# fab-jul/imgcomp-cvpr

Hardware: AMD Instinct MI355X
Metric: Megapixels/s encode+pc-logits (and decode) per node (higher is better)
Workload: dtype f32

## Files before the change

### imgcomp_cvpr_amd/csrc/conv3x3_wino4.hip

```cpp
#include "wino_common.h"
#include "internal.h"

#define W4_QUADS 9
#define W4_PACKED_FLOATS (36 * WN_C * WN_C)
#define W4_ACC_A 32
#ifndef W4_RA
#define W4_RA 9
#endif
#ifndef W4_RB
#define W4_RB 3
#endif
#ifndef W4_TURN
#define W4_TURN 6
#endif
#ifndef W4_GAP
#define W4_GAP 10
#endif
#ifndef W4_PRE_N
#define W4_PRE_N 2
#endif
#ifndef W4_PRE
#define W4_PRE 31
#endif
#ifndef W4_WT_MAX
#define W4_WT_MAX 512
#endif
#ifndef W4_ABL
#define W4_ABL 0
#endif
#ifndef W4_SLICE1
#define W4_SLICE1 1
#endif
#ifndef W4_SOFT
#define W4_SOFT 0
#endif
#ifndef W4_WG8_FLAGS
#define W4_WG8_FLAGS 1
#endif
#define W4_WG8_SPINS (1 << 16)
#define W4_B1 29
#define W4_B2 8
#ifndef W4_SPREAD
#define W4_SPREAD 1
#endif

__device__ __forceinline__ int w4_tap5(int mode, int phase, int a) {
    if (mode == 2) return phase ? 2 * a : (a == 0 ? -1 : 2 * a - 1);
    return phase ? 4 - 2 * a : (a == 2 ? -1 : 3 - 2 * a);
}
__global__ __launch_bounds__(256) void wino4_pack_kernel(const float* __restrict__ w_tf, const float* const* __restrict__ w_tab, float* __restrict__ out,
                                                        int mode, int CI, int CO) {
    const int idx = blockIdx.x * 256 + threadIdx.x;
    if (idx >= CI * CO) return;
    if (w_tab) { w_tf = w_tab[blockIdx.y]; out += (size_t)blockIdx.y * 36 * CI * CO; }
    const int cin = idx / CO, cout = idx % CO;
    double g[3][3];
#pragma unroll
    for (int a = 0; a < 3; ++a)
#pragma unroll
        for (int b = 0; b < 3; ++b) {
            if (mode == 0) g[a][b] = (double)w_tf[((a * 3 + b) * WN_C + cin) * WN_C + cout];
            else if (mode == 1) g[a][b] = (double)w_tf[(((2 - a) * 3 + (2 - b)) * WN_C + cout) * WN_C + cin];
            else if (mode == 2) {
                const int ph = cin >> 6, c = cin & 63, ky = w4_tap5(2, ph >> 1, a), kx = w4_tap5(2, ph & 1, b);
                g[a][b] = (ky < 0 || kx < 0) ? 0.0 : (double)w_tf[((ky * 5 + kx) * 64 + c) * 128 + cout];
            } else {
                const int ph = cout & 3, c = cout >> 2, ky = w4_tap5(3, ph >> 1, a), kx = w4_tap5(3, ph & 1, b);
                g[a][b] = (ky < 0 || kx < 0) ? 0.0 : (double)w_tf[((ky * 5 + kx) * 64 + c) * 128 + cin];
            }
        }
    const double G[6][3] = {{0.25, 0.0, 0.0}, {-1.0 / 6, -1.0 / 6, -1.0 / 6}, {-1.0 / 6, 1.0 / 6, -1.0 / 6},
                            {1.0 / 24, 1.0 / 12, 1.0 / 6}, {1.0 / 24, -1.0 / 12, 1.0 / 6}, {0.0, 0.0, 1.0}};
    double t[6][3];
#pragma unroll
    for (int x = 0; x < 6; ++x)
#pragma unroll
        for (int b = 0; b < 3; ++b) t[x][b] = G[x][0] * g[0][b] + G[x][1] * g[1][b] + G[x][2] * g[2][b];
    float* o = out + ((size_t)((cout >> 4) * (CI >> 2) + (cin >> 2)) * W4_QUADS * 64 + ((cin & 3) * 16 + (cout & 15))) * 4;
#pragma unroll
    for (int x = 0; x < 6; ++x)
#pragma unroll
        for (int v = 0; v < 6; ++v) {
            const int p = 6 * x + v;
            o[(p >> 2) * 256 + (p & 3)] = (float)(t[x][0] * G[v][0] + t[x][1] * G[v][1] + t[x][2] * G[v][2]);
        }
}

extern "C" size_t ic_wino4_3x3_c128_packed_floats(void) { return W4_PACKED_FLOATS; }

extern "C" int ic_pack_wino4_3x3_c128_f32(const float* w_tf, float* w_packed, int backward, ic_stream_t stream) {
    IC_CHECK_ARG(w_tf && w_packed);
    hipLaunchKernelGGL(wino4_pack_kernel, dim3(WN_C * WN_C / 256), dim3(256), 0, (hipStream_t)stream, w_tf, nullptr, w_packed, backward ? 1 : 0, WN_C, WN_C);
    IC_LAUNCH_CHECK();
    return IC_OK;
}

extern "C" int ic_pack_wino4_3x3_c128_batch_f32(const float* const* w_tf_table_dev, float* w_packed, int layers, int backward, ic_stream_t stream) {
    IC_CHECK_ARG(w_tf_table_dev && w_packed && layers > 0);
    hipLaunchKernelGGL(wino4_pack_kernel, dim3(WN_C * WN_C / 256, layers), dim3(256), 0, (hipStream_t)stream, nullptr, w_tf_table_dev, w_packed,
                       backward ? 1 : 0, WN_C, WN_C);
    IC_LAUNCH_CHECK();
    return IC_OK;
}

extern "C" size_t ic_wino4_conv5s2_packed_floats(void) { return (size_t)36 * 256 * 128; }

extern "C" int ic_pack_wino4_conv5s2_f32(const float* w_tf, float* w_packed, int transposed, ic_stream_t stream) {
    IC_CHECK_ARG(w_tf && w_packed);
    hipLaunchKernelGGL(wino4_pack_kernel, dim3(256 * 128 / 256), dim3(256), 0, (hipStream_t)stream, w_tf, nullptr, w_packed, transposed ? 3 : 2,
                       transposed ? 128 : 256, transposed ? 256 : 128);
    IC_LAUNCH_CHECK();
    return IC_OK;
}

__device__ __forceinline__ void w4_bt(const float d0, const float d1, const float d2, const float d3, const float d4, const float d5,
                                      float& t0, float& t1, float& t2, float& t3, float& t4, float& t5) {
    const float p = fmaf(-4.f, d2, d4), q = fmaf(-4.f, d1, d3);
    const float r = d4 - d2, s = 2.f * (d3 - d1);
    const float a0 = fmaf(4.f, d0, fmaf(-5.f, d2, d4));
    const float a5 = fmaf(4.f, d1, fmaf(-5.f, d3, d5));
    t0 = a0;
    t1 = p + q;
    t2 = p - q;
    t3 = r + s;
    t4 = r - s;
    t5 = a5;
}
__device__ __forceinline__ void w4_at(float m0, float m1, float m2, float m3, float m4, float m5,
                                      float& y0, float& y1, float& y2, float& y3) {
    const float s1 = m1 + m2, d1 = m1 - m2, s2 = m3 + m4, d2 = m3 - m4;
    y0 = (m0 + s1) + s2;
    y1 = fmaf(2.f, d2, d1);
    y2 = fmaf(4.f, s2, s1);
    y3 = fmaf(8.f, d2, d1) + m5;
}

template <bool WT, int RES, int CIN, int COUT, bool SHUF, bool SEG2, bool WG8, bool STATS = false>
__global__ __launch_bounds__(WG8 ? 512 : 256) __attribute__((amdgpu_waves_per_eu(2, 2)))
void wino4_3x3_kernel(const WnArgs a) {
    constexpr int WAVES = WG8 ? 8 : 4;
    constexpr int KS = CIN / 4, IT = KS / 4, PARTS = COUT / (16 * WAVES);
    __shared__ f32x4 ring[2 * 4 * W4_QUADS * 64];
    __shared__ float pf_sink[64];
    __shared__ unsigned w8_flag[4];
#ifdef W4_STAMPS
    const unsigned long long t_entry = __builtin_amdgcn_s_memtime();
#endif
#ifdef W4_LAUNCH_STAMPS
    const unsigned long long ls_c0 = __builtin_amdgcn_s_memtime(), ls_r0 = __builtin_amdgcn_s_memrealtime();
#endif
    const int wave = __builtin_amdgcn_readfirstlane(threadIdx.x >> 6);
    const int lane = threadIdx.x & 63, n16 = lane & 15, kq = lane >> 4;
    const int b = a.xcd_runs ? ic_xcd_run(blockIdx.x, gridDim.x) : (int)blockIdx.x;
    const int part = b % PARTS;
    const int seg = b / PARTS + a.g0;
    const int sx = seg % a.gcols, t_ = seg / a.gcols;
    const int ty = t_ % a.grows, n = t_ / a.grows;
    const int cot = part * WAVES + wave;
    const int pw = wave & 3;
    const int grp = WG8 ? wave >> 2 : 0;
    const int hrow = SEG2 ? (n16 >> 3) : 0;
    const int tx = SEG2 ? 8 * sx + (n16 & 7) : 16 * sx + n16;
    const int H = a.H, W = a.W, HW = H * W;

    const __amdgpu_buffer_rsrc_t xr = __builtin_amdgcn_make_buffer_rsrc((void*)(a.x + (size_t)n * CIN * HW), 0, CIN * HW * 4, 0x00020000);
    const __amdgpu_buffer_rsrc_t fr = __builtin_amdgcn_make_buffer_rsrc((void*)a.wp, 0, 36 * CIN * COUT * 4, 0x00020000);
    const bool col_ok = 4 * tx < W;
    const bool first_lane = SEG2 ? (n16 & 7) == 0 : n16 == 0, last_lane = SEG2 ? (n16 & 7) == 7 : n16 == 15;
    const bool mid_l = SEG2 && n16 == 8, mid_r = SEG2 && n16 == 7;
    const int ecol = first_lane ? 4 * tx - 1 : (last_lane ? 4 * tx + 4 : -1);
    const bool e_ok = col_ok && ecol >= 0 && ecol < W;
    const int tyr = SEG2 ? 2 * ty : ty;
    const int r_first = 4 * tyr - 1;
    const int obase = (kq * HW + (r_first + 4 * hrow) * W + 4 * tx) * 4;
    const int ebase = (kq * HW + (r_first + 4 * hrow) * W + ecol) * 4;
    const unsigned fo = (unsigned)lane * 16u;

    f32x4 acc[36];
#pragma unroll
    for (int p = 0; p < 36; ++p) acc[p] = f32x4{0.f, 0.f, 0.f, 0.f};
#pragma unroll
    for (int p = 0; p < 36; ++p) {
        if (p < W4_ACC_A) asm volatile("" : "+a"(acc[p]));
        else asm volatile("" : "+v"(acc[p]));
    }
    __builtin_amdgcn_sched_barrier(0);

    typedef __attribute__((address_space(3))) f32x4 lds_f32x4;
    unsigned rb1 = (unsigned)(size_t)&ring[4 * W4_QUADS * 64 + lane];
    if (WG8) asm volatile("" : "+v"(rb1));
    auto ring_rd = [&](int half, int idx) __attribute__((always_inline)) -> f32x4 {
        if (WG8 && half) return *(reinterpret_cast<lds_f32x4*>((size_t)rb1) + idx * 64);
        return ring[(half * 4 * W4_QUADS + idx) * 64 + lane];
    };

    f32x4 pr[6];
    float pe[6];
    auto load_patch = [&](int ks) __attribute__((always_inline)) {
        const int so = ks * 4 * HW * 4;
        int ob = obase, eb = ebase;
        asm volatile("" : "+v"(ob), "+v"(eb));
#pragma unroll
        for (int i = 0; i < 6; ++i) {
            const bool row_lo = r_first + i >= 0 && r_first + i < H;
            const bool row_hi = r_first + 4 + i < H;
            const bool row_ok = SEG2 ? (hrow ? row_hi : row_lo) : row_lo;
            const unsigned o1 = (row_ok && col_ok) ? (unsigned)(ob + i * W * 4) : WN_OOB;
            const unsigned o2 = (row_ok && e_ok) ? (unsigned)(eb + i * W * 4) : WN_OOB;
            pr[i] = __builtin_bit_cast(f32x4, __builtin_amdgcn_raw_buffer_load_b128(xr, o1, so, 0));
            pe[i] = __builtin_bit_cast(float, __builtin_amdgcn_raw_buffer_load_b32(xr, o2, so, 0));
        }
    };
    auto transform_put = [&](int half) __attribute__((always_inline)) {
        float u[6][6];
#pragma unroll
        for (int i = 0; i < 6; ++i) {
            u[i][0] = dpp_from_left(pe[i], pr[i][3]);
            u[i][5] = dpp_from_right(pe[i], pr[i][0]);
            if (SEG2) { u[i][0] = mid_l ? pe[i] : u[i][0]; u[i][5] = mid_r ? pe[i] : u[i][5]; }
            u[i][1] = pr[i][0]; u[i][2] = pr[i][1]; u[i][3] = pr[i][2]; u[i][4] = pr[i][3];
        }
        __builtin_amdgcn_sched_barrier(0);
#pragma unroll
        for (int j = 0; j < 6; ++j) {
            w4_bt(u[0][j], u[1][j], u[2][j], u[3][j], u[4][j], u[5][j], u[0][j], u[1][j], u[2][j], u[3][j], u[4][j], u[5][j]);
            __builtin_amdgcn_sched_barrier(0);
        }
        f32x4* dst = &ring[((half * 4 + pw) * W4_QUADS) * 64 + lane];
#pragma unroll
        for (int x = 0; x < 6; x += 2) {
            float v0[6], v1[6];
            w4_bt(u[x][0], u[x][1], u[x][2], u[x][3], u[x][4], u[x][5], v0[0], v0[1], v0[2], v0[3], v0[4], v0[5]);
            w4_bt(u[x + 1][0], u[x + 1][1], u[x + 1][2], u[x + 1][3], u[x + 1][4], u[x + 1][5], v1[0], v1[1], v1[2], v1[3], v1[4], v1[5]);
            const int q0 = 3 * (x / 2);
            dst[(q0 + 0) * 64] = f32x4{v0[0], v0[1], v0[2], v0[3]};
            dst[(q0 + 1) * 64] = f32x4{v0[4], v0[5], v1[0], v1[1]};
            dst[(q0 + 2) * 64] = f32x4{v1[2], v1[3], v1[4], v1[5]};
            __builtin_amdgcn_sched_barrier(0);
        }
    };
    float su[6][6], sp = 0.f, sq = 0.f, sr = 0.f, se = 0.f, sa = 0.f, sh4 = 0.f, sh5 = 0.f;
    auto bt_first = [&](float d0, float d1, float d2, float d3, float d4) __attribute__((always_inline)) {
        sp = fmaf(-4.f, d2, d4); sq = fmaf(-4.f, d1, d3); sr = d4 - d2; se = d3 - d1;
        sa = fmaf(4.f, d0, fmaf(-5.f, d2, d4));
    };
    auto bt_second = [&](float d1, float d3, float d5, float& t0, float& t1, float& t2, float& t3, float& t4, float& t5) __attribute__((always_inline)) {
        const float a5 = fmaf(4.f, d1, fmaf(-5.f, d3, d5));
        t0 = sa; t1 = sp + sq; t2 = sp - sq; t3 = fmaf(2.f, se, sr); t4 = fmaf(-2.f, se, sr); t5 = a5;
    };
    auto slice = [&](int k, int part, int half) __attribute__((always_inline)) {
        if (k == 0) {
#pragma unroll
            for (int i = 0; i < 6; ++i) {
                if (part == 0) {
                    su[i][0] = dpp_from_left(pe[i], pr[i][3]);
                    if (SEG2) su[i][0] = mid_l ? pe[i] : su[i][0];
                } else {
                    su[i][5] = dpp_from_right(pe[i], pr[i][0]);
                    if (SEG2) su[i][5] = mid_r ? pe[i] : su[i][5];
                    su[i][1] = pr[i][0]; su[i][2] = pr[i][1]; su[i][3] = pr[i][2]; su[i][4] = pr[i][3];
                }
            }
        } else if (k <= 6) {
            const int c = k == 1 ? 0 : (k == 2 ? 5 : k - 2);
            if (part == 0) bt_first(su[0][c], su[1][c], su[2][c], su[3][c], su[4][c]);
            else bt_second(su[1][c], su[3][c], su[5][c], su[0][c], su[1][c], su[2][c], su[3][c], su[4][c], su[5][c]);
        } else {
            const int x = k - 7;
            if (part == 0) bt_first(su[x][0], su[x][1], su[x][2], su[x][3], su[x][4]);
            else {
                float v[6];
                bt_second(su[x][1], su[x][3], su[x][5], v[0], v[1], v[2], v[3], v[4], v[5]);
                f32x4* dst = &ring[((half * 4 + pw) * W4_QUADS + 3 * (x / 2)) * 64 + lane];
                if ((x & 1) == 0) { dst[0] = f32x4{v[0], v[1], v[2], v[3]}; sh4 = v[4]; sh5 = v[5]; }
                else { dst[64] = f32x4{sh4, sh5, v[0], v[1]}; dst[128] = f32x4{v[2], v[3], v[4], v[5]}; }
            }
        }
    };
    auto kill_patch = [&]() __attribute__((always_inline)) {
#pragma unroll
        for (int i = 0; i < 6; ++i) { asm volatile("" : "=v"(pr[i])); asm volatile("" : "=v"(pe[i])); }
    };
    auto kill_slices = [&]() __attribute__((always_inline)) {
#pragma unroll
        for (int i = 0; i < 6; ++i)
#pragma unroll
            for (int jx = 0; jx < 6; ++jx) asm volatile("" : "=v"(su[i][jx]));
        asm volatile("" : "=v"(sp)); asm volatile("" : "=v"(sq)); asm volatile("" : "=v"(sr)); asm volatile("" : "=v"(se));
        asm volatile("" : "=v"(sa)); asm volatile("" : "=v"(sh4)); asm volatile("" : "=v"(sh5));
    };
    const unsigned w8_base = (unsigned)(size_t)w8_flag;
    auto flag_add = [&](int k) __attribute__((always_inline)) {
        asm volatile("s_mov_b64 exec, 1\n\tds_add_u32 %0, %1\n\ts_mov_b64 exec, -1" :: "v"(w8_base + 4u * k), "v"(1u) : "memory");
    };
    auto flag_wait = [&](int k, unsigned target) __attribute__((always_inline)) {
        unsigned v, sv, spins;
        asm volatile("s_mov_b32 %2, 0\n"
                     "1:\tds_read_b32 %0, %3\n\t"
                     "s_waitcnt lgkmcnt(0)\n\t"
                     "v_readfirstlane_b32 %1, %0\n\t"
                     "s_add_u32 %2, %2, 1\n\t"
                     "s_cmp_ge_u32 %1, %4\n\t"
                     "s_cbranch_scc1 2f\n\t"
                     "s_cmp_lt_u32 %2, %5\n\t"
                     "s_cbranch_scc1 1b\n"
                     "2:"
                     : "=&v"(v), "=&s"(sv), "=&s"(spins) : "v"(w8_base + 4u * k), "s"(target), "i"(W4_WG8_SPINS) : "memory", "scc");
    };
    f32x4 fa[W4_RA];
    auto load_filter = [&](int slot, int Q) __attribute__((always_inline)) {
        fa[slot] = __builtin_bit_cast(f32x4, __builtin_amdgcn_raw_buffer_load_b128(fr, fo, (cot * KS * W4_QUADS + Q) * 1024, 0));
    };

    const int img_bytes = COUT * HW * 4;
    f32x4 e1a[4], e1b[4];
    float scv[4], shv[4];
#pragma unroll
    for (int i = 0; i < 4; ++i) { e1a[i] = e1b[i] = f32x4{0.f, 0.f, 0.f, 0.f}; scv[i] = shv[i] = 0.f; }
    auto epilogue_lanes = [&](unsigned* lo, int& kq_e) __attribute__((always_inline)) {
        int lane_e = (int)__builtin_amdgcn_mbcnt_hi(~0u, __builtin_amdgcn_mbcnt_lo(~0u, 0u));
        asm volatile("" : "+v"(lane_e));
        kq_e = lane_e >> 4;
        const int tx_e = SEG2 ? 8 * sx + (lane_e & 7) : 16 * sx + (lane_e & 15);
        const bool col_ok_e = 4 * tx_e < W;
#pragma unroll
        for (int i = 0; i < 4; ++i) {
            const int oy = 4 * (SEG2 ? 2 * ty + ((lane_e >> 3) & 1) : ty) + i;
            lo[i] = (col_ok_e && oy < H) ? (unsigned)((4 * kq_e * HW + oy * W + 4 * tx_e) * 4) : WN_OOB;
        }
    };
    auto request_first = [&](int first, int count) __attribute__((always_inline)) {
        unsigned lo[4];
        int kq_e;
        epilogue_lanes(lo, kq_e);
        if (first == 0 && !STATS) {
#pragma unroll
            for (int r = 0; r < 4; ++r) {
                const int ch = SHUF ? 4 * cot + kq_e : 16 * cot + 4 * kq_e + r;
                scv[r] = a.scale[ch]; shv[r] = a.shift[ch];
            }
        }
        if (RES > 0) {
            const __amdgpu_buffer_rsrc_t r1r = __builtin_amdgcn_make_buffer_rsrc((void*)(a.res1 ? a.res1 + (size_t)n * COUT * HW : a.x), 0, a.res1 ? img_bytes : 0, 0x00020000);
#pragma unroll
            for (int i = 0; i < 4; ++i) {
                if (first == 0) e1a[i] = __builtin_bit_cast(f32x4, __builtin_amdgcn_raw_buffer_load_b128(r1r, lo[i], 16 * cot * HW * 4, 0));
                if (first + count > 1) e1b[i] = __builtin_bit_cast(f32x4, __builtin_amdgcn_raw_buffer_load_b128(r1r, lo[i], (16 * cot + 1) * HW * 4, 0));
            }
        }
    };

    if (!WG8 || grp == 0) load_patch(pw);
#pragma unroll
    for (int Q = 0; Q < W4_RA - 1; ++Q) load_filter(Q, Q);
    if (a.wp_next) {
        constexpr unsigned LINES = 36u * CIN * COUT * 4u / 128u;
        const unsigned n_x = (gridDim.x + 7u) >> 3, j_x = blockIdx.x >> 3;
        const unsigned per = (LINES + n_x - 1) / n_x, l0 = j_x * per;
        const __amdgpu_buffer_rsrc_t nr = __builtin_amdgcn_make_buffer_rsrc((void*)a.wp_next, 0, 36 * CIN * COUT * 4, 0x00020000);
        const unsigned sink = (unsigned)(size_t)pf_sink;
        for (unsigned l = threadIdx.x; l < per; l += 64 * WAVES) {
            const unsigned off = (l0 + l) < LINES ? (l0 + l) * 128u : WN_OOB;
            unsigned keep;
            asm volatile("s_mov_b32 %0, m0\n\ts_mov_b32 m0, %3\n\ts_nop 0\n\tbuffer_load_dword %1, %2, 0 offen lds\n\ts_mov_b32 m0, %0"
                         : "=&s"(keep) : "v"(off), "s"(nr), "s"(sink) : "memory");
        }
    }
    if (!WG8 || grp == 0) transform_put(0);
    if (WG8 && W4_WG8_FLAGS && threadIdx.x < 4) w8_flag[threadIdx.x] = 0u;
    asm volatile("s_waitcnt lgkmcnt(0)" ::: "memory");
    __builtin_amdgcn_s_barrier();

#ifdef W4_STAMPS
    const unsigned long long t_loop0 = __builtin_amdgcn_s_memtime();
#endif
    f32x4 bq[W4_RB];
#pragma unroll
    for (int q0 = 0; q0 < W4_RB - 1; ++q0) bq[q0] = ring_rd(0, q0);
    auto iteration = [&](const int j, const int u2, const bool last, const bool produce) __attribute__((always_inline)) {
        if (WG8 && W4_WG8_FLAGS && j > 0) flag_wait(u2, 4u * ((unsigned)(j + 1) >> 1));
        if (!W4_SOFT && j > 0) {
#pragma unroll
            for (int q0 = 0; q0 < W4_RB - 1; ++q0) bq[q0] = ring_rd(u2, q0);
        }
#pragma unroll
        for (int lq = 0; lq < 36; ++lq) {
            const int q = lq % W4_QUADS;
            const int Q = j * 36 + lq;
            const int sk = lq - (W4_TURN + W4_GAP);
#pragma unroll
            for (int i = 0; i < 4; ++i) {
                if (4 * q + i < W4_ACC_A) asm volatile("v_mfma_f32_16x16x4_f32 %0, %1, %2, %0" : "+a"(acc[4 * q + i]) : "v"(fa[lq % W4_RA][i]), "v"(bq[lq % W4_RB][i]));
                else asm volatile("v_mfma_f32_16x16x4_f32 %0, %1, %2, %0" : "+v"(acc[4 * q + i]) : "v"(fa[lq % W4_RA][i]), "v"(bq[lq % W4_RB][i]));
                if (WG8 && !last && sk == 0 && i == 0) kill_slices();
                if (W4_SPREAD && produce && !(W4_ABL & 4) && i < (W4_SLICE1 ? 1 : 2) && sk >= 0 && sk < 13) {
                    __builtin_amdgcn_sched_barrier(0);
                    if (WG8 && W4_WG8_FLAGS && sk == 7 && i == 0) flag_wait(2 + (u2 ^ 1), 8u * ((unsigned)(j + 1) >> 1));
                    slice(sk, i, u2 ^ 1);
                    if (W4_SLICE1) slice(sk, 1, u2 ^ 1);
                    if (WG8 && W4_WG8_FLAGS && sk == 12 && i == (W4_SLICE1 ? 0 : 1)) flag_add(u2 ^ 1);
                    __builtin_amdgcn_sched_barrier(0);
                }
            }
#if W4_ABL & 1
            if ((lq & 1) == 0)
#endif
            if (!last || lq + W4_RA - 1 < 36) load_filter((lq + W4_RA - 1) % W4_RA, Q + W4_RA - 1);
            {
                const int ah = lq + W4_RB - 1;
                if (ah < 36 && !((W4_ABL & 2) && (lq & 1)))
                    bq[ah % W4_RB] = ring_rd(u2, ah);
                else if (W4_SOFT && !last) bq[ah % W4_RB] = ring_rd(u2 ^ 1, ah - 36);
            }
            if (WG8 && !last && lq == W4_TURN) kill_patch();
            if (lq == W4_TURN && produce) load_patch(4 * (j + 1) + pw);
            if (!W4_SPREAD && lq == W4_TURN + W4_GAP && produce) transform_put(u2 ^ 1);
            if (last && lq == W4_PRE) request_first(0, W4_PRE_N);
            if (W4_SOFT && !last && lq == W4_B1) {
                asm volatile("s_waitcnt lgkmcnt(0)" ::: "memory");
                __builtin_amdgcn_s_barrier();
            }
            if (W4_SOFT && !last && lq == W4_B2 && j > 0) __builtin_amdgcn_s_barrier();
            if (WG8 && W4_WG8_FLAGS && !last && lq == 36 - W4_RB + 1) flag_add(2 + u2);
            __builtin_amdgcn_sched_barrier(0);
        }
        if (!W4_SOFT && !(WG8 && W4_WG8_FLAGS)) {
            asm volatile("s_waitcnt lgkmcnt(0)" ::: "memory");
            __builtin_amdgcn_s_barrier();
        }
    };
    for (int jj = 0; jj < IT - 2; jj += 2) {
        iteration(jj, 0, false, !WG8 || grp == 1);
        iteration(jj + 1, 1, false, !WG8 || grp == 0);
    }
    iteration(IT - 2, 0, false, !WG8 || grp == 1);
    iteration(IT - 1, 1, true, false);
#ifdef W4_STAMPS
    const unsigned long long t_loop1 = __builtin_amdgcn_s_memtime();
#endif

    asm volatile("s_nop 15\n\ts_nop 15" ::: "memory");
#pragma unroll
    for (int p = 0; p < 36; ++p) {
        if (p < W4_ACC_A) asm volatile("" : "+a"(acc[p]));
        else asm volatile("" : "+v"(acc[p]));
    }

    if (W4_PRE < 0) request_first(0, 2);
    else if (W4_PRE_N < 2) request_first(1, 1);
    unsigned lo[4];
    int kq_e;
    epilogue_lanes(lo, kq_e);
    const float relu_lo = a.relu ? 0.f : -__builtin_inff();
    auto out_tile = [&](int r, float (&y)[4][4]) __attribute__((always_inline)) {
        float w_[6][4];
#pragma unroll
        for (int x = 0; x < 6; ++x) {
#pragma unroll
            for (int v = 0; v < 6; ++v) {
                if (6 * x + v < W4_ACC_A) asm volatile("" : "+a"(acc[6 * x + v]));
                else asm volatile("" : "+v"(acc[6 * x + v]));
            }
            w4_at(acc[6 * x][r], acc[6 * x + 1][r], acc[6 * x + 2][r], acc[6 * x + 3][r], acc[6 * x + 4][r], acc[6 * x + 5][r],
                  w_[x][0], w_[x][1], w_[x][2], w_[x][3]);
            __builtin_amdgcn_sched_barrier(0);
        }
#pragma unroll
        for (int jx = 0; jx < 4; ++jx) {
            w4_at(w_[0][jx], w_[1][jx], w_[2][jx], w_[3][jx], w_[4][jx], w_[5][jx], y[0][jx], y[1][jx], y[2][jx], y[3][jx]);
            __builtin_amdgcn_sched_barrier(0);
        }
    };
    if (SHUF) {
        const __amdgpu_buffer_rsrc_t yr = __builtin_amdgcn_make_buffer_rsrc((void*)(a.y + (size_t)n * COUT * HW), 0, img_bytes, 0x00020000);
        int lane_s = (int)__builtin_amdgcn_mbcnt_hi(~0u, __builtin_amdgcn_mbcnt_lo(~0u, 0u));
        asm volatile("" : "+v"(lane_s));
        const int tx_s = SEG2 ? 8 * sx + (lane_s & 7) : 16 * sx + (lane_s & 15);
        const int ty_s = SEG2 ? 2 * ty + ((lane_s >> 3) & 1) : ty;
        const bool col_ok_s = 4 * tx_s < W;
        const int so = 4 * cot * 4 * HW * 4;
#pragma unroll
        for (int py = 0; py < 2; ++py) {
            f32x4 o0[4], o1[4];
            {
                float y[4][4];
                out_tile(2 * py, y);
#pragma unroll
                for (int i = 0; i < 4; ++i) {
#pragma unroll
                    for (int jx = 0; jx < 4; ++jx) o0[i][jx] = fmaxf(fmaf(y[i][jx], scv[0], shv[0]), relu_lo);
                    asm volatile("" : "+v"(o0[i]));
                }
            }
            __builtin_amdgcn_sched_barrier(0);
            {
                float y[4][4];
                out_tile(2 * py + 1, y);
#pragma unroll
                for (int i = 0; i < 4; ++i) {
#pragma unroll
                    for (int jx = 0; jx < 4; ++jx) o1[i][jx] = fmaxf(fmaf(y[i][jx], scv[0], shv[0]), relu_lo);
                }
            }
            __builtin_amdgcn_sched_barrier(0);
#pragma unroll
            for (int i = 0; i < 4; ++i) {
                const int oy = 4 * ty_s + i;
                const unsigned lo_s = (col_ok_s && oy < H) ? (unsigned)(((lane_s >> 4) * 4 * HW + (2 * oy + py) * 2 * W + 8 * tx_s) * 4) : WN_OOB;
                const f32x4 oa = f32x4{o0[i][0], o1[i][0], o0[i][1], o1[i][1]}, ob = f32x4{o0[i][2], o1[i][2], o0[i][3], o1[i][3]};
                __builtin_amdgcn_raw_buffer_store_b128(__builtin_bit_cast(u32x4, oa), yr, lo_s, so, WT ? 16 : 0);
                __builtin_amdgcn_raw_buffer_store_b128(__builtin_bit_cast(u32x4, ob), yr, lo_s + 16u, so, WT ? 16 : 0);
            }
            __builtin_amdgcn_sched_barrier(0);
        }
    } else {
    const __amdgpu_buffer_rsrc_t yr = __builtin_amdgcn_make_buffer_rsrc((void*)(a.y + (size_t)n * COUT * HW), 0, img_bytes, 0x00020000);
    const __amdgpu_buffer_rsrc_t r1r = __builtin_amdgcn_make_buffer_rsrc((void*)(a.res1 ? a.res1 + (size_t)n * COUT * HW : a.x), 0, a.res1 ? img_bytes : 0, 0x00020000);
    const __amdgpu_buffer_rsrc_t r2r = __builtin_amdgcn_make_buffer_rsrc((void*)(a.res2 ? a.res2 + (size_t)n * COUT * HW : a.x), 0, a.res2 ? img_bytes : 0, 0x00020000);
    constexpr bool has1 = RES >= 1, has2 = RES >= 2;
#pragma unroll
    for (int r = 0; r < 4; ++r) {
        const int co = 16 * cot + r;
        const int so = co * HW * 4;
        f32x4 e2[4];
#pragma unroll
        for (int i = 0; i < 4; ++i)
            e2[i] = has2 ? __builtin_bit_cast(f32x4, __builtin_amdgcn_raw_buffer_load_b128(r2r, lo[i], so, 0)) : f32x4{0.f, 0.f, 0.f, 0.f};
        float y[4][4];
        out_tile(r, y);
        f32x4 o[4];
#pragma unroll
        for (int i = 0; i < 4; ++i) {
#pragma unroll
            for (int jx = 0; jx < 4; ++jx) o[i][jx] = STATS ? y[i][jx] : fmaxf(fmaf(y[i][jx], scv[r], shv[r]), relu_lo);
            if (has1) o[i] += (r & 1) ? e1b[i] : e1a[i];
            if (has2) o[i] += e2[i];
        }
        if (STATS) {
            float s0 = 0.f, s1 = 0.f;
#pragma unroll
            for (int i = 0; i < 4; ++i) {
                const bool ok = lo[i] != WN_OOB;
#pragma unroll
                for (int jx = 0; jx < 4; ++jx) { const float v = ok ? o[i][jx] : 0.f; s0 += v; s1 = fmaf(v, v, s1); }
            }
#define W4_ROW_SHR_ADD(v, n) v += __int_as_float(__builtin_amdgcn_update_dpp(0, __float_as_int(v), 0x110 + (n), 0xf, 0xf, true))
            W4_ROW_SHR_ADD(s0, 1); W4_ROW_SHR_ADD(s1, 1);
            W4_ROW_SHR_ADD(s0, 2); W4_ROW_SHR_ADD(s1, 2);
            W4_ROW_SHR_ADD(s0, 4); W4_ROW_SHR_ADD(s1, 4);
            W4_ROW_SHR_ADD(s0, 8); W4_ROW_SHR_ADD(s1, 8);
#undef W4_ROW_SHR_ADD
            int lane_t = (int)__builtin_amdgcn_mbcnt_hi(~0u, __builtin_amdgcn_mbcnt_lo(~0u, 0u));
            if ((lane_t & 15) == 15) {
                float* d = a.stats + ((size_t)(co + 4 * (lane_t >> 4)) * a.ngroups + (seg - a.g0)) * 2;
                d[0] = s0; d[1] = s1;
            }
        }
        __builtin_amdgcn_sched_barrier(0);
        if (has1 && r + 2 < 4) {
#pragma unroll
            for (int i = 0; i < 4; ++i) {
                const f32x4 v = __builtin_bit_cast(f32x4, __builtin_amdgcn_raw_buffer_load_b128(r1r, lo[i], so + 2 * HW * 4, 0));
                if (r & 1) e1b[i] = v; else e1a[i] = v;
            }
        }
        __builtin_amdgcn_sched_barrier(0);
#pragma unroll
        for (int i = 0; i < 4; ++i)
            __builtin_amdgcn_raw_buffer_store_b128(__builtin_bit_cast(u32x4, o[i]), yr, lo[i], so, WT ? 16 : 0);
        __builtin_amdgcn_sched_barrier(0);
    }
    }
#ifdef W4_LAUNCH_STAMPS
    if (a.prof && (threadIdx.x & 63) == 0) {
        asm volatile("s_waitcnt vmcnt(0)" ::: "memory");
        const unsigned long long ls_c1 = __builtin_amdgcn_s_memtime(), ls_r1 = __builtin_amdgcn_s_memrealtime();
        unsigned long long* d = a.prof + 4 * ((size_t)blockIdx.x * WAVES + (threadIdx.x >> 6));
        d[0] = ls_r0; d[1] = ls_r1; d[2] = ls_c1 - ls_c0; d[3] = (unsigned long long)(36 * KS);
    }
#endif
#ifdef W4_STAMPS
    if (a.prof && (threadIdx.x & 63) == 0) {
        asm volatile("s_waitcnt vmcnt(0)" ::: "memory");
        unsigned long long* d = a.prof + 6 * ((size_t)blockIdx.x * WAVES + (threadIdx.x >> 6));
        const unsigned long long t_end = __builtin_amdgcn_s_memtime();
        d[0] = t_loop0 - t_entry; d[1] = t_loop1 - t_loop0; d[2] = t_end - t_loop1; d[3] = t_entry; d[4] = t_end;
        d[5] = (unsigned long long)__builtin_amdgcn_s_getreg(0xF804) | ((unsigned long long)__builtin_amdgcn_s_getreg(0xF814) << 32);
    }
#endif
}

#ifdef W4_STAMPS
static void* g_w4_dbg = nullptr;
extern "C" void ic_wino4_debug_set_buffer(void* p) { g_w4_dbg = p; }
#endif
#ifdef W4_LAUNCH_STAMPS
#include <atomic>
static unsigned long long* g_w4_ls = nullptr;
static long long g_w4_ls_cap = 0, g_w4_ls_max_launches = 0;
static std::atomic<long long> g_w4_ls_next{0}, g_w4_ls_launch{0};
static long long* g_w4_ls_table = nullptr;
extern "C" void ic_wino4_launch_stamps_set(void* dev_records, long long capacity_waves, long long* host_table, long long max_launches) {
    g_w4_ls = (unsigned long long*)dev_records; g_w4_ls_cap = capacity_waves; g_w4_ls_table = host_table; g_w4_ls_max_launches = max_launches;
    g_w4_ls_next = 0; g_w4_ls_launch = 0;
}
extern "C" long long ic_wino4_launch_stamps_count(void) { return g_w4_ls_launch.load(); }
#endif

extern "C" int ic_wino4_3x3_c128_supported(int N, int H, int W) {
    return N > 0 && H > 0 && W > 0 && (W & 3) == 0 && (long long)WN_C * H * W * 4 < (1ll << 31);
}

static inline long long w4_segments(int H, int W, bool seg2) {
    const long long th = ic_cdiv(H, 4), tw = ic_cdiv(W, 4);
    return seg2 ? ((th + 1) / 2) * ((tw + 7) / 8) : th * ((tw + 15) / 16);
}
static inline bool w4_seg2(int H, int W) { return w4_segments(H, W, true) < w4_segments(H, W, false); }

extern "C" long long ic_wino4_3x3_c128_workgroups(int N, int H, int W) {
    if (!ic_wino4_3x3_c128_supported(N, H, W)) return 0;
    return 2ll * N * w4_segments(H, W, w4_seg2(H, W));
}

extern "C" int ic_wino4_3x3_c128_waves(int N, int H, int W, int flags) {
    if (!ic_wino4_3x3_c128_supported(N, H, W)) return 0;
    if ((flags & IC_CONV3_WINO4_WG4) || w4_seg2(H, W)) return 4;
    if (flags & IC_CONV3_WINO4_WG8) return 8;
    return ic_wino4_3x3_c128_workgroups(N, H, W) >= 2048 ? 8 : 4;
}

template <int RES, int CIN, int COUT, bool SHUF, bool SEG2, bool WG8>
static int w4_launch2(const float* x, const float* w_packed, const float* scale, const float* shift, const float* res1, const float* res2,
                      float* y, int N, int H, int W, int relu, int flags, hipStream_t st, const float* w_next = nullptr) {
    WnArgs a{};
    a.x = x; a.wp = w_packed; a.wp_next = w_next; a.scale = scale; a.shift = shift; a.res1 = res1; a.res2 = res2; a.y = y;
    a.N = N; a.H = H; a.W = W; a.relu = relu;
    a.grows = SEG2 ? ic_cdiv(ic_cdiv(H, 4), 2) : ic_cdiv(H, 4);
    a.gcols = SEG2 ? ic_cdiv(W, 32) : ic_cdiv(W, 64);
    a.xcd_runs = (flags & IC_CONV3_NO_XCD_RUNS) ? 0 : 1;
    a.g0 = 0; a.ngroups = N * a.grows * a.gcols;
#ifdef W4_STAMPS
    a.prof = (unsigned long long*)g_w4_dbg;
#endif
    constexpr int WAVES = WG8 ? 8 : 4;
    const long long wgs = (long long)(COUT / (16 * WAVES)) * a.ngroups;
#ifdef W4_LAUNCH_STAMPS
    if (g_w4_ls) {
        const long long first = g_w4_ls_next.fetch_add(WAVES * wgs), l = g_w4_ls_launch.load();
        if (first + WAVES * wgs <= g_w4_ls_cap && l < g_w4_ls_max_launches) {
            g_w4_ls_launch.fetch_add(1);
            a.prof = g_w4_ls + 4 * first;
            g_w4_ls_table[3 * l] = first; g_w4_ls_table[3 * l + 1] = WAVES * wgs; g_w4_ls_table[3 * l + 2] = CIN * 1000 + COUT;
        }
    }
#endif
    const dim3 grid((unsigned)wgs), block(64 * WAVES);
    if (wgs * WAVES <= W4_WT_MAX * 4) hipLaunchKernelGGL((wino4_3x3_kernel<true, RES, CIN, COUT, SHUF, SEG2, WG8>), grid, block, 0, st, a);
    else hipLaunchKernelGGL((wino4_3x3_kernel<false, RES, CIN, COUT, SHUF, SEG2, WG8>), grid, block, 0, st, a);
    IC_LAUNCH_CHECK();
    return IC_OK;
}
template <int RES, int CIN, int COUT, bool SHUF>
static int w4_launch(const float* x, const float* w_packed, const float* scale, const float* shift, const float* res1, const float* res2,
                     float* y, int N, int H, int W, int relu, int flags, hipStream_t st, const float* w_next = nullptr) {
    if (CIN == 128 && COUT == 128 && ic_wino4_3x3_c128_waves(N, H, W, flags) == 8) {
        constexpr bool r = CIN == 128 && COUT == 128;
        return w4_launch2<RES, CIN, COUT, SHUF, false, r>(x, w_packed, scale, shift, res1, res2, y, N, H, W, relu, flags, st, w_next);
    }
    if (w4_seg2(H, W)) return w4_launch2<RES, CIN, COUT, SHUF, true, false>(x, w_packed, scale, shift, res1, res2, y, N, H, W, relu, flags, st, w_next);
    return w4_launch2<RES, CIN, COUT, SHUF, false, false>(x, w_packed, scale, shift, res1, res2, y, N, H, W, relu, flags, st, w_next);
}

int icx_wino4_3x3_c128_next(const float* x, const float* w_packed, const float* scale, const float* shift, const float* res1, const float* res2,
                            float* y, int N, int H, int W, int relu, int flags, const float* w_packed_next, hipStream_t st) {
    IC_CHECK_ARG(x && w_packed && scale && shift && y);
    IC_CHECK_ARG(N > 0 && H > 0 && W > 0);
    if (!ic_wino4_3x3_c128_supported(N, H, W)) return IC_ERR_UNSUPPORTED;
    if (res2) return w4_launch<2, 128, 128, false>(x, w_packed, scale, shift, res1, res2, y, N, H, W, relu, flags, st, w_packed_next);
    return w4_launch<1, 128, 128, false>(x, w_packed, scale, shift, res1, nullptr, y, N, H, W, relu, flags, st, w_packed_next);
}
extern "C" long long ic_wino4_3x3_c128_stats_parts(int N, int H, int W) {
    if (!ic_wino4_3x3_c128_supported(N, H, W)) return 0;
    return (long long)N * w4_segments(H, W, w4_seg2(H, W));
}
template <bool SEG2>
static int w4_launch_stats(const float* x, const float* w_packed, float* y, float* stats, int N, int H, int W, int flags, hipStream_t st) {
    WnArgs a{};
    a.x = x; a.wp = w_packed; a.y = y; a.stats = stats;
    a.N = N; a.H = H; a.W = W; a.relu = 0;
    a.grows = SEG2 ? ic_cdiv(ic_cdiv(H, 4), 2) : ic_cdiv(H, 4);
    a.gcols = SEG2 ? ic_cdiv(W, 32) : ic_cdiv(W, 64);
    a.xcd_runs = (flags & IC_CONV3_NO_XCD_RUNS) ? 0 : 1;
    a.g0 = 0; a.ngroups = N * a.grows * a.gcols;
    const long long wgs = 2ll * a.ngroups;
    const dim3 grid((unsigned)wgs), block(256);
    if (wgs <= W4_WT_MAX) hipLaunchKernelGGL((wino4_3x3_kernel<true, 0, 128, 128, false, SEG2, false, true>), grid, block, 0, st, a);
    else hipLaunchKernelGGL((wino4_3x3_kernel<false, 0, 128, 128, false, SEG2, false, true>), grid, block, 0, st, a);
    IC_LAUNCH_CHECK();
    return IC_OK;
}
extern "C" int ic_wino4_3x3_c128_raw_stats_f32(const float* x, const float* w_packed, float* y, float* stats, int N, int H, int W,
                                               int flags, ic_stream_t stream) {
    IC_CHECK_ARG(x && w_packed && y && stats && N > 0 && H > 0 && W > 0);
    if (!ic_wino4_3x3_c128_supported(N, H, W)) return IC_ERR_UNSUPPORTED;
    if (w4_seg2(H, W)) return w4_launch_stats<true>(x, w_packed, y, stats, N, H, W, flags, (hipStream_t)stream);
    return w4_launch_stats<false>(x, w_packed, y, stats, N, H, W, flags, (hipStream_t)stream);
}

extern "C" int ic_wino4_3x3_c128_bn_act_f32(const float* x, const float* w_packed, const float* scale, const float* shift,
                                            const float* res1, const float* res2, float* y, int N, int H, int W, int relu,
                                            int flags, ic_stream_t stream) {
    return icx_wino4_3x3_c128_next(x, w_packed, scale, shift, res1, res2, y, N, H, W, relu, flags, nullptr, (hipStream_t)stream);
}

extern "C" int ic_wino4_conv5s2_supported(int N, int H, int W) {
    return N > 0 && H > 0 && W > 0 && (W & 3) == 0 && (long long)256 * H * W * 4 < (1ll << 31);
}
extern "C" long long ic_wino4_conv5s2_workgroups(int N, int H, int W, int transposed) {
    if (!ic_wino4_conv5s2_supported(N, H, W)) return 0;
    return (transposed ? 4ll : 2ll) * N * w4_segments(H, W, w4_seg2(H, W));
}
extern "C" int ic_wino4_conv5s2_c64_c128_bn_act_f32(const float* x_phases, const float* w_packed, const float* scale, const float* shift,
                                                    float* y, int N, int H, int W, int relu, int flags, ic_stream_t stream) {
    IC_CHECK_ARG(x_phases && w_packed && scale && shift && y);
    if (!ic_wino4_conv5s2_supported(N, H, W)) return IC_ERR_UNSUPPORTED;
    return w4_launch<0, 256, 128, false>(x_phases, w_packed, scale, shift, nullptr, nullptr, y, N, H, W, relu, flags, (hipStream_t)stream);
}
extern "C" int ic_wino4_deconv5s2_c128_c64_bn_act_f32(const float* x, const float* w_packed, const float* scale, const float* shift,
                                                      float* y, int N, int H, int W, int relu, int flags, ic_stream_t stream) {
    IC_CHECK_ARG(x && w_packed && scale && shift && y);
    if (!ic_wino4_conv5s2_supported(N, H, W)) return IC_ERR_UNSUPPORTED;
    return w4_launch<0, 128, 256, true>(x, w_packed, scale, shift, nullptr, nullptr, y, N, H, W, relu, flags, (hipStream_t)stream);
}

__global__ __launch_bounds__(256) void space_to_depth2_kernel(const float* __restrict__ x, float* __restrict__ y, int C, int H, int W, long long total) {
    for (long long i = (long long)blockIdx.x * 256 + threadIdx.x; i < total; i += (long long)gridDim.x * 256) {
        const int w = (int)(i % W); long long t = i / W;
        const int h = (int)(t % H); t /= H;
        const int c = (int)(t % C); t /= C;
        const int ph = (int)(t & 3); const long long n = t >> 2;
        y[i] = x[((n * C + c) * 2 * H + 2 * h + (ph >> 1)) * 2 * W + 2 * w + (ph & 1)];
    }
}
extern "C" int ic_space_to_depth2_f32(const float* x, float* y, int N, int C, int H2, int W2, ic_stream_t stream) {
    IC_CHECK_ARG(x && y && N > 0 && C > 0 && H2 > 0 && W2 > 0 && !(H2 & 1) && !(W2 & 1));
    const long long total = (long long)N * C * H2 * W2;
    const long long g = (total + 255) / 256;
    hipLaunchKernelGGL(space_to_depth2_kernel, dim3((unsigned)(g > 4096 ? 4096 : g)), dim3(256), 0, (hipStream_t)stream, x, y, C, H2 / 2, W2 / 2, total);
    IC_LAUNCH_CHECK();
    return IC_OK;
}
```

Measured before the change: 244.1.

## Cut Winograd F(4x4) kernel VGPR and setup overhead in accumulator and load paths

Moves all accumulators from AGPRs to VGPRs by default, and drops the explicit zero-init loop: the first K-iteration now issues MFMAs with a zero C operand. The input buffer descriptor is shifted back one row so row offsets go into the scalar soffset. In the non-SEG2 path, out-of-range rows are handled by swapping in a zero-size descriptor rather than a per-lane offset select. The horizontal B^T transform of the edge column now runs before the DPP neighbour exchange, so only transformed values are shuffled and fewer raw-pixel registers stay live. These changes aim to reduce VALU work, register pressure and initialisation cost, but they change register allocation and the slice schedule in ways that could spill or stall.

```diff
diff --git a/imgcomp_cvpr_amd/csrc/conv3x3_wino4.hip b/imgcomp_cvpr_amd/csrc/conv3x3_wino4.hip
--- a/imgcomp_cvpr_amd/csrc/conv3x3_wino4.hip
+++ b/imgcomp_cvpr_amd/csrc/conv3x3_wino4.hip
@@ -3,7 +3,9 @@
 
 #define W4_QUADS 9
 #define W4_PACKED_FLOATS (36 * WN_C * WN_C)
-#define W4_ACC_A 32
+#ifndef W4_ACC_A
+#define W4_ACC_A 0
+#endif
 #ifndef W4_RA
 #define W4_RA 9
 #endif
@@ -163,7 +165,9 @@
     const int tx = SEG2 ? 8 * sx + (n16 & 7) : 16 * sx + n16;
     const int H = a.H, W = a.W, HW = H * W;
 
-    const __amdgpu_buffer_rsrc_t xr = __builtin_amdgcn_make_buffer_rsrc((void*)(a.x + (size_t)n * CIN * HW), 0, CIN * HW * 4, 0x00020000);
+    const float* xb = a.x + (size_t)n * CIN * HW - W;
+    const __amdgpu_buffer_rsrc_t xr = __builtin_amdgcn_make_buffer_rsrc((void*)xb, 0, (CIN * HW + W) * 4, 0x00020000);
+    const __amdgpu_buffer_rsrc_t xz = __builtin_amdgcn_make_buffer_rsrc((void*)xb, 0, 0, 0x00020000);
     const __amdgpu_buffer_rsrc_t fr = __builtin_amdgcn_make_buffer_rsrc((void*)a.wp, 0, 36 * CIN * COUT * 4, 0x00020000);
     const bool col_ok = 4 * tx < W;
     const bool first_lane = SEG2 ? (n16 & 7) == 0 : n16 == 0, last_lane = SEG2 ? (n16 & 7) == 7 : n16 == 15;
@@ -172,19 +176,11 @@
     const bool e_ok = col_ok && ecol >= 0 && ecol < W;
     const int tyr = SEG2 ? 2 * ty : ty;
     const int r_first = 4 * tyr - 1;
-    const int obase = (kq * HW + (r_first + 4 * hrow) * W + 4 * tx) * 4;
-    const int ebase = (kq * HW + (r_first + 4 * hrow) * W + ecol) * 4;
+    const unsigned obase = col_ok ? (unsigned)((kq * HW + 4 * hrow * W + 4 * tx) * 4) : WN_OOB;
+    const unsigned ebase = e_ok ? (unsigned)((kq * HW + 4 * hrow * W + ecol) * 4) : WN_OOB;
     const unsigned fo = (unsigned)lane * 16u;
 
     f32x4 acc[36];
-#pragma unroll
-    for (int p = 0; p < 36; ++p) acc[p] = f32x4{0.f, 0.f, 0.f, 0.f};
-#pragma unroll
-    for (int p = 0; p < 36; ++p) {
-        if (p < W4_ACC_A) asm volatile("" : "+a"(acc[p]));
-        else asm volatile("" : "+v"(acc[p]));
-    }
-    __builtin_amdgcn_sched_barrier(0);
 
     typedef __attribute__((address_space(3))) f32x4 lds_f32x4;
     unsigned rb1 = (unsigned)(size_t)&ring[4 * W4_QUADS * 64 + lane];
@@ -197,35 +193,42 @@
     f32x4 pr[6];
     float pe[6];
     auto load_patch = [&](int ks) __attribute__((always_inline)) {
-        const int so = ks * 4 * HW * 4;
-        int ob = obase, eb = ebase;
-        asm volatile("" : "+v"(ob), "+v"(eb));
+        const int so = (ks * 4 * HW + (r_first + 1) * W) * 4;
+        unsigned ob = obase, eb = ebase;
+        if (SEG2) asm volatile("" : "+v"(ob), "+v"(eb));
 #pragma unroll
         for (int i = 0; i < 6; ++i) {
             const bool row_lo = r_first + i >= 0 && r_first + i < H;
             const bool row_hi = r_first + 4 + i < H;
-            const bool row_ok = SEG2 ? (hrow ? row_hi : row_lo) : row_lo;
-            const unsigned o1 = (row_ok && col_ok) ? (unsigned)(ob + i * W * 4) : WN_OOB;
-            const unsigned o2 = (row_ok && e_ok) ? (unsigned)(eb + i * W * 4) : WN_OOB;
-            pr[i] = __builtin_bit_cast(f32x4, __builtin_amdgcn_raw_buffer_load_b128(xr, o1, so, 0));
-            pe[i] = __builtin_bit_cast(float, __builtin_amdgcn_raw_buffer_load_b32(xr, o2, so, 0));
+            if (SEG2) {
+                const bool row_ok = hrow ? row_hi : row_lo;
+                pr[i] = __builtin_bit_cast(f32x4, __builtin_amdgcn_raw_buffer_load_b128(xr, row_ok ? ob : WN_OOB, so + i * W * 4, 0));
+                pe[i] = __builtin_bit_cast(float, __builtin_amdgcn_raw_buffer_load_b32(xr, row_ok ? eb : WN_OOB, so + i * W * 4, 0));
+            } else {
+                const __amdgpu_buffer_rsrc_t xi = row_lo ? xr : xz;
+                pr[i] = __builtin_bit_cast(f32x4, __builtin_amdgcn_raw_buffer_load_b128(xi, ob, so + i * W * 4, 0));
+                pe[i] = __builtin_bit_cast(float, __builtin_amdgcn_raw_buffer_load_b32(xi, eb, so + i * W * 4, 0));
+            }
         }
     };
     auto transform_put = [&](int half) __attribute__((always_inline)) {
         float u[6][6];
 #pragma unroll
-        for (int i = 0; i < 6; ++i) {
-            u[i][0] = dpp_from_left(pe[i], pr[i][3]);
-            u[i][5] = dpp_from_right(pe[i], pr[i][0]);
-            if (SEG2) { u[i][0] = mid_l ? pe[i] : u[i][0]; u[i][5] = mid_r ? pe[i] : u[i][5]; }
-            u[i][1] = pr[i][0]; u[i][2] = pr[i][1]; u[i][3] = pr[i][2]; u[i][4] = pr[i][3];
-        }
+        for (int i = 0; i < 6; ++i) { u[i][1] = pr[i][0]; u[i][2] = pr[i][1]; u[i][3] = pr[i][2]; u[i][4] = pr[i][3]; }
+        w4_bt(pe[0], pe[1], pe[2], pe[3], pe[4], pe[5], pe[0], pe[1], pe[2], pe[3], pe[4], pe[5]);
         __builtin_amdgcn_sched_barrier(0);
 #pragma unroll
-        for (int j = 0; j < 6; ++j) {
+        for (int j = 1; j < 5; ++j) {
             w4_bt(u[0][j], u[1][j], u[2][j], u[3][j], u[4][j], u[5][j], u[0][j], u[1][j], u[2][j], u[3][j], u[4][j], u[5][j]);
             __builtin_amdgcn_sched_barrier(0);
         }
+#pragma unroll
+        for (int i = 0; i < 6; ++i) {
+            u[i][0] = dpp_from_left(pe[i], u[i][4]);
+            u[i][5] = dpp_from_right(pe[i], u[i][1]);
+            if (SEG2) { u[i][0] = mid_l ? pe[i] : u[i][0]; u[i][5] = mid_r ? pe[i] : u[i][5]; }
+        }
+        __builtin_amdgcn_sched_barrier(0);
         f32x4* dst = &ring[((half * 4 + pw) * W4_QUADS) * 64 + lane];
 #pragma unroll
         for (int x = 0; x < 6; x += 2) {
@@ -250,21 +253,27 @@
     };
     auto slice = [&](int k, int part, int half) __attribute__((always_inline)) {
         if (k == 0) {
+            if (part == 0) {
+#pragma unroll
+                for (int i = 0; i < 6; ++i) { su[i][1] = pr[i][0]; su[i][2] = pr[i][1]; su[i][3] = pr[i][2]; su[i][4] = pr[i][3]; }
+                bt_first(pe[0], pe[1], pe[2], pe[3], pe[4]);
+            } else bt_second(pe[1], pe[3], pe[5], pe[0], pe[1], pe[2], pe[3], pe[4], pe[5]);
+        } else if (k == 3) {
 #pragma unroll
             for (int i = 0; i < 6; ++i) {
                 if (part == 0) {
-                    su[i][0] = dpp_from_left(pe[i], pr[i][3]);
+                    su[i][0] = dpp_from_left(pe[i], su[i][4]);
                     if (SEG2) su[i][0] = mid_l ? pe[i] : su[i][0];
                 } else {
-                    su[i][5] = dpp_from_right(pe[i], pr[i][0]);
+                    su[i][5] = dpp_from_right(pe[i], su[i][1]);
                     if (SEG2) su[i][5] = mid_r ? pe[i] : su[i][5];
-                    su[i][1] = pr[i][0]; su[i][2] = pr[i][1]; su[i][3] = pr[i][2]; su[i][4] = pr[i][3];
                 }
             }
-        } else if (k <= 6) {
-            const int c = k == 1 ? 0 : (k == 2 ? 5 : k - 2);
+        } else if (k < 6) {
+            const int c = k == 1 ? 1 : (k == 2 ? 4 : k - 2);
             if (part == 0) bt_first(su[0][c], su[1][c], su[2][c], su[3][c], su[4][c]);
             else bt_second(su[1][c], su[3][c], su[5][c], su[0][c], su[1][c], su[2][c], su[3][c], su[4][c], su[5][c]);
+        } else if (k == 6) {
         } else {
             const int x = k - 7;
             if (part == 0) bt_first(su[x][0], su[x][1], su[x][2], su[x][3], su[x][4]);
@@ -377,7 +386,7 @@
     f32x4 bq[W4_RB];
 #pragma unroll
     for (int q0 = 0; q0 < W4_RB - 1; ++q0) bq[q0] = ring_rd(0, q0);
-    auto iteration = [&](const int j, const int u2, const bool last, const bool produce) __attribute__((always_inline)) {
+    auto iteration = [&](const int j, const int u2, const bool last, const bool produce, const bool first = false) __attribute__((always_inline)) {
         if (WG8 && W4_WG8_FLAGS && j > 0) flag_wait(u2, 4u * ((unsigned)(j + 1) >> 1));
         if (!W4_SOFT && j > 0) {
 #pragma unroll
@@ -390,7 +399,10 @@
             const int sk = lq - (W4_TURN + W4_GAP);
 #pragma unroll
             for (int i = 0; i < 4; ++i) {
-                if (4 * q + i < W4_ACC_A) asm volatile("v_mfma_f32_16x16x4_f32 %0, %1, %2, %0" : "+a"(acc[4 * q + i]) : "v"(fa[lq % W4_RA][i]), "v"(bq[lq % W4_RB][i]));
+                if (first && lq < W4_QUADS) {
+                    if (4 * q + i < W4_ACC_A) asm volatile("v_mfma_f32_16x16x4_f32 %0, %1, %2, 0" : "=&a"(acc[4 * q + i]) : "v"(fa[lq % W4_RA][i]), "v"(bq[lq % W4_RB][i]));
+                    else asm volatile("v_mfma_f32_16x16x4_f32 %0, %1, %2, 0" : "=&v"(acc[4 * q + i]) : "v"(fa[lq % W4_RA][i]), "v"(bq[lq % W4_RB][i]));
+                } else if (4 * q + i < W4_ACC_A) asm volatile("v_mfma_f32_16x16x4_f32 %0, %1, %2, %0" : "+a"(acc[4 * q + i]) : "v"(fa[lq % W4_RA][i]), "v"(bq[lq % W4_RB][i]));
                 else asm volatile("v_mfma_f32_16x16x4_f32 %0, %1, %2, %0" : "+v"(acc[4 * q + i]) : "v"(fa[lq % W4_RA][i]), "v"(bq[lq % W4_RB][i]));
                 if (WG8 && !last && sk == 0 && i == 0) kill_slices();
                 if (W4_SPREAD && produce && !(W4_ABL & 4) && i < (W4_SLICE1 ? 1 : 2) && sk >= 0 && sk < 13) {
@@ -429,7 +441,9 @@
             __builtin_amdgcn_s_barrier();
         }
     };
-    for (int jj = 0; jj < IT - 2; jj += 2) {
+    iteration(0, 0, false, !WG8 || grp == 1, true);
+    iteration(1, 1, false, !WG8 || grp == 0);
+    for (int jj = 2; jj < IT - 2; jj += 2) {
         iteration(jj, 0, false, !WG8 || grp == 1);
         iteration(jj + 1, 1, false, !WG8 || grp == 0);
     }
@@ -608,7 +622,7 @@
 #endif
 
 extern "C" int ic_wino4_3x3_c128_supported(int N, int H, int W) {
-    return N > 0 && H > 0 && W > 0 && (W & 3) == 0 && (long long)WN_C * H * W * 4 < (1ll << 31);
+    return N > 0 && H > 0 && W > 0 && (W & 3) == 0 && ((long long)WN_C * H * W + W) * 4 < (1ll << 31);
 }
 
 static inline long long w4_segments(int H, int W, bool seg2) {
@@ -714,7 +728,7 @@
 }
 
 extern "C" int ic_wino4_conv5s2_supported(int N, int H, int W) {
-    return N > 0 && H > 0 && W > 0 && (W & 3) == 0 && (long long)256 * H * W * 4 < (1ll << 31);
+    return N > 0 && H > 0 && W > 0 && (W & 3) == 0 && ((long long)256 * H * W + W) * 4 < (1ll << 31);
 }
 extern "C" long long ic_wino4_conv5s2_workgroups(int N, int H, int W, int transposed) {
     if (!ic_wino4_conv5s2_supported(N, H, W)) return 0;
```

Result: faster. 248.2, median of 6 (+1.7%).
